# olga24912/lodestar

Hardware: AMD Instinct MI355X
Metric: verified signature sets/sec (node) (higher is better)
Workload: dtype u32/u64 (28-bit-limb Montgomery integer arithmetic); 1 GPU; C2 gossip attestation flood: 16384 single-pubkey sets per GPU, 1 set per batchable job; pk_mode=device table, sig_encoding=compressed 96 B, distinct_messages=16384, group_sets=1024, group_policy=0, inflight=32, slots=3, hw_queues=4, merge_sets=131072, pipeline_depth=3, parallelism=shard-by-job x1 (in-process devices), no collective

## Files before the change

lodestar_amd/build.py:

```python
import hashlib
import os
import subprocess
import sys
import time

PKG = os.path.dirname(os.path.abspath(__file__))
ROOT = os.path.dirname(PKG)
CSRC = os.path.join(PKG, "csrc")
LIB = os.environ.get("BLSGPU_LIB") or os.path.join(PKG, "libblsgpu.so")
ARCH = os.environ.get("BLSGPU_ARCH", "gfx950")
HIPCC = os.environ.get("HIPCC", "/opt/rocm/bin/hipcc")
SOURCES = ["k_sig.hip", "k_msm.hip", "k_hash.hip", "k_hmap.hip", "k_pk.hip", "k_sigagg.hip", "k_awr.hip", "k_same.hip", "k_aggverify.hip", "k_miller.hip", "k_group.hip", "k_inv.hip", "k_ssz.hip", "k_debug.hip", "k_tower_debug.hip",
           "runtime.cpp", "pipeline.cpp", "helpers.cpp"]


OBJ_DIR = os.path.join(PKG, "build")


TU_DEFINES = {"k_sig.hip": ["BLS_INLINE_BIG=1"]}


def tu_defines():
    env = os.environ.get("BLSGPU_TU_DEFINES")
    if env is None:
        return TU_DEFINES
    out = {}
    for part in filter(None, env.split(";")):
        tu, _, defs = part.partition("=")
        out[tu] = [d for d in defs.split("+") if d]
    return out


_ILP = ["-mllvm", "-amdgpu-sched-strategy=max-ilp"]
_MINREG = ["-mllvm", "-amdgpu-sched-strategy=iterative-minreg"]
TU_CFLAGS = {"k_hash.hip": _MINREG, "k_pk.hip": _ILP}


def tu_cflags():
    env = os.environ.get("BLSGPU_TU_CFLAGS")
    if env is None:
        return TU_CFLAGS
    out = {}
# ... 103 lines not shown
```

lodestar_amd/csrc/hash_to_curve.hpp:

```cpp
#pragma once
#include "curve.hpp"

BLS_CONST uint32_t SHA256_K[64] = {
    0x428a2f98, 0x71374491, 0xb5c0fbcf, 0xe9b5dba5, 0x3956c25b, 0x59f111f1, 0x923f82a4, 0xab1c5ed5,
    0xd807aa98, 0x12835b01, 0x243185be, 0x550c7dc3, 0x72be5d74, 0x80deb1fe, 0x9bdc06a7, 0xc19bf174,
    0xe49b69c1, 0xefbe4786, 0x0fc19dc6, 0x240ca1cc, 0x2de92c6f, 0x4a7484aa, 0x5cb0a9dc, 0x76f988da,
    0x983e5152, 0xa831c66d, 0xb00327c8, 0xbf597fc7, 0xc6e00bf3, 0xd5a79147, 0x06ca6351, 0x14292967,
    0x27b70a85, 0x2e1b2138, 0x4d2c6dfc, 0x53380d13, 0x650a7354, 0x766a0abb, 0x81c2c92e, 0x92722c85,
    0xa2bfe8a1, 0xa81a664b, 0xc24b8b70, 0xc76c51a3, 0xd192e819, 0xd6990624, 0xf40e3585, 0x106aa070,
    0x19a4c116, 0x1e376c08, 0x2748774c, 0x34b0bcb5, 0x391c0cb3, 0x4ed8aa4a, 0x5b9cca4f, 0x682e6ff3,
    0x748f82ee, 0x78a5636f, 0x84c87814, 0x8cc70208, 0x90befffa, 0xa4506ceb, 0xbef9a3f7, 0xc67178f2};
BLS_CONST uint32_t SHA256_IV[8] = {0x6a09e667, 0xbb67ae85, 0x3c6ef372, 0xa54ff53a,
                                   0x510e527f, 0x9b05688c, 0x1f83d9ab, 0x5be0cd19};

BLS_HD uint32_t rotr32(uint32_t x, int n) { return (x >> n) | (x << (32 - n)); }

struct sha_st {
  uint32_t h[8];
};
struct sha_blk {
  uint32_t w[16];
};
BLS_HDNI sha_st sha256_block(sha_st st, sha_blk blk) {
  uint32_t a = st.h[0], b = st.h[1], c = st.h[2], d = st.h[3], e = st.h[4], f = st.h[5], g = st.h[6], h = st.h[7];
// ... 106 lines not shown
    int bit = 32 * k;
    int li = bit / BLS_LB, off = bit % BLS_LB;
    lim[li] |= (v << off) & BLS_MASK;
    if (li + 1 < 19) lim[li + 1] |= (off == 0) ? (v >> BLS_LB) : ((v >> (BLS_LB - off)) & BLS_MASK);
    if (off > 0 && li + 2 < 19 && (32 - (BLS_LB - off)) > BLS_LB) lim[li + 2] |= v >> (2 * BLS_LB - off);
  }
  fp lo, hi;
#pragma unroll
  for (int i = 0; i < BLS_NL; i++) lo.l[i] = lim[i];
#pragma unroll
  for (int i = 0; i < BLS_NL; i++) hi.l[i] = (i < 5) ? lim[BLS_NL + i] : 0;
  return fp_add(fp_mul(lo, FP_R2), fp_mul(hi, FP_R3));
}

BLS_INL void hash_to_field_fp2x2(const uint8_t msg[32], fp2& u0, fp2& u1) {
  uint32_t ub[64];
  expand_message_xmd_32(msg, ub);
  u0.c0 = fp_from_be64_words(ub + 0);
  u0.c1 = fp_from_be64_words(ub + 16);
  u1.c0 = fp_from_be64_words(ub + 32);
  u1.c1 = fp_from_be64_words(ub + 48);
}

BLS_INL fp2 fp2_sqrt_with_normroot(const fp2& a, const fp& s) {
  fp t = fp_half(fp_add(a.c0, s));
  fp t_alt = fp_half(fp_sub(a.c0, s));
  t = fp_select(fp_is_zero(t), t_alt, t);
  fp y = fp_pow_p34(t);
  fp x0 = fp_mul(t, y);
  fp a1y2 = fp_half(fp_mul(a.c1, y));
  bool res_case = fp_eq(fp_sqr(x0), t);
  fp2 r;
  r.c0 = fp_select(res_case, x0, a1y2);
  r.c1 = fp_select(res_case, a1y2, fp_neg(x0));
  return r;
}

BLS_HD fp2 fp2_plain(const fp2& a) { return fp2_make(fp_from_mont(a.c0), fp_from_mont(a.c1)); }

BLS_INL g2a sswu_map(const fp2& u, const fp2& Zu2, const fp2& tv, const fp2& tv_inv) {
  fp2 x1 = fp2_mul(SSWU_MINUS_B_OVER_A, fp2_add(fp2_one(), tv_inv));
  x1 = fp2_select(fp2_is_zero(tv), SSWU_B_OVER_ZA, x1);
  fp2 gx1 = fp2_add(fp2_mul(fp2_add(fp2_sqr(x1), SSWU_A), x1), SSWU_B);
  fp2 x2 = fp2_mul(Zu2, x1);
  fp2 gx2 = fp2_add(fp2_mul(fp2_add(fp2_sqr(x2), SSWU_A), x2), SSWU_B);
  fp n1 = fp2_norm(gx1);
  fp s1 = fp_mul(n1, fp_pow_p34(n1));
  bool sq1 = fp_eq(fp_sqr(s1), n1);
  fp nu = fp2_norm(u);
  fp s2 = fp_mul(fp_mul(SSWU_C125, s1), fp_mul(fp_sqr(nu), nu));
  fp2 g = fp2_select(sq1, gx1, gx2);
  fp2 x = fp2_select(sq1, x1, x2);
  fp s = fp_select(sq1, s1, s2);
  fp2 y = fp2_sqrt_with_normroot(g, s);
  fp2 up = fp2_plain(u);
  fp2 yp = fp2_plain(y);
  uint32_t su = fp2_sgn0_plain(up.c0, up.c1);
  uint32_t sy = fp2_sgn0_plain(yp.c0, yp.c1);
  y = fp2_select(su != sy, fp2_neg(y), y);
  g2a r;
  r.x = x;
  r.y = y;
  return r;
}

BLS_INL g2j iso3_map_jac(const g2a& p) {
  const fp2& x = p.x;
  fp2 x2 = fp2_sqr(x);
  fp2 x3 = fp2_mul(x2, x);
  fp2 Nx = fp2_add(fp2_add(fp2_mul(ISO_XNUM_3, x3), fp2_mul(ISO_XNUM_2, x2)), fp2_add(fp2_mul(ISO_XNUM_1, x), ISO_XNUM_0));
  fp2 Dx = fp2_add(fp2_add(x2, fp2_mul(ISO_XDEN_1, x)), ISO_XDEN_0);
  fp2 Ny = fp2_add(fp2_add(fp2_mul(ISO_YNUM_3, x3), fp2_mul(ISO_YNUM_2, x2)), fp2_add(fp2_mul(ISO_YNUM_1, x), ISO_YNUM_0));
  fp2 Dy = fp2_add(fp2_add(x3, fp2_mul(ISO_YDEN_2, x2)), fp2_add(fp2_mul(ISO_YDEN_1, x), ISO_YDEN_0));
  g2j r;
  fp2 DxDy = fp2_mul(Dx, Dy);
  r.z = DxDy;
  r.x = fp2_mul(fp2_mul(Nx, Dy), DxDy);
  fp2 Dx2 = fp2_sqr(Dx);
  r.y = fp2_mul(fp2_mul(fp2_mul(p.y, Ny), fp2_mul(Dx2, Dx)), fp2_sqr(Dy));
  if (fp2_is_zero(DxDy)) r = jac_infinity<fp2>();
  return r;
}

BLS_HDNI g2j clear_cofactor_g2(const g2j& P) {
  g2j t1 = jac_neg(jac_mul_zabs(P));
  g2j t2 = g2_psi(P);
// ... 16 lines not shown
    st(2, jac_add(jac_add(g2_psi2(jac_dbl(P)), jac_neg(psiP)), jac_add(A, jac_neg(P))));
  }
  const jac<F> D = jac_mul_zabs_ld<F>([&] { return ld(1); });
  return jac_add(D, ld(2));
}
template <class Ld, class St>
BLS_INL g2j clear_cofactor_g2_slots(Ld ld, St st) {
  return clear_cofactor_slots<fp2>(ld, st);
}

struct h2c_prep {
  fp2 u0, u1, Zu2_0, Zu2_1, tv0, tv1, d;
};
BLS_INL void hash_to_g2_prep(const uint8_t msg[32], h2c_prep& h) {
  hash_to_field_fp2x2(msg, h.u0, h.u1);
  h.Zu2_0 = fp2_mul(SSWU_Z, fp2_sqr(h.u0));
  h.Zu2_1 = fp2_mul(SSWU_Z, fp2_sqr(h.u1));
  h.tv0 = fp2_add(fp2_sqr(h.Zu2_0), h.Zu2_0);
  h.tv1 = fp2_add(fp2_sqr(h.Zu2_1), h.Zu2_1);
  const fp2 a0 = fp2_select(fp2_is_zero(h.tv0), fp2_one(), h.tv0);
  const fp2 a1 = fp2_select(fp2_is_zero(h.tv1), fp2_one(), h.tv1);
  h.d = fp2_mul(a0, a1);
}
BLS_INL g2j hash_to_g2_map_j(const h2c_prep& h, const fp2& dinv, int j) {
  const bool z0 = fp2_is_zero(h.tv0), z1 = fp2_is_zero(h.tv1);
  const fp2 a_other = j == 0 ? fp2_select(z1, fp2_one(), h.tv1) : fp2_select(z0, fp2_one(), h.tv0);
  const bool zj = j == 0 ? z0 : z1;
  const fp2 inv = fp2_select(zj, fp2_zero(), fp2_mul(dinv, a_other));
  const bool j0 = j == 0;
  const g2a q = sswu_map(fp2_select(j0, h.u0, h.u1), fp2_select(j0, h.Zu2_0, h.Zu2_1), fp2_select(j0, h.tv0, h.tv1), inv);
  return iso3_map_jac(q);
}

BLS_HDNI g2j hash_to_g2_finish(const h2c_prep& h, const fp2& dinv) {
  const bool z0 = fp2_is_zero(h.tv0), z1 = fp2_is_zero(h.tv1);
  const fp2 a0 = fp2_select(z0, fp2_one(), h.tv0);
  const fp2 a1 = fp2_select(z1, fp2_one(), h.tv1);
  const fp2 inv0 = fp2_select(z0, fp2_zero(), fp2_mul(dinv, a1));
  const fp2 inv1 = fp2_select(z1, fp2_zero(), fp2_mul(dinv, a0));
  g2a q0 = sswu_map(h.u0, h.Zu2_0, h.tv0, inv0);
  g2a q1 = sswu_map(h.u1, h.Zu2_1, h.tv1, inv1);
  g2j Q = jac_add(iso3_map_jac(q0), iso3_map_jac(q1));
  return clear_cofactor_g2(Q);
}

BLS_HDNI g2j hash_to_g2_jac(const uint8_t msg[32]) {
  h2c_prep h;
  hash_to_g2_prep(msg, h);
  return hash_to_g2_finish(h, fp2_inv(h.d));
}
```

lodestar_amd/csrc/helpers.cpp:

```cpp
#include "aggverify_plan.hpp"
#include "helper_layout.hpp"
#include "runtime_internal.hpp"

using namespace blsgpu_rt;
namespace hl = helper_layout;
namespace avp = aggverify_plan;

static_assert(hl::kFp == W_FP && hl::kG1A == W_G1A && hl::kG1J == W_G1J && hl::kG2A == W_G2A && hl::kG2J == W_G2J &&
                  hl::kFp12 == W_FP12 && hl::kAwrTabWords == AWR_TAB_WORDS && hl::kMillerLineWords == kMillerLineWords,
              "helper_layout.hpp restates the element widths of kernels.h");

namespace {

template <class Body>
int helper_call(blsgpu_ctx* ctx, bool reads_table, Body body) {
  if (!enter(ctx)) return BLSGPU_ERR_CLOSED;
  struct Leave {
    blsgpu_ctx* ctx;
    ~Leave() { leave(ctx); }
  } leave_on_exit{ctx};
  Device& d = *ctx->devs[0];
  try {
    std::lock_guard<std::mutex> helper(d.helper_mu);
    std::shared_lock<std::shared_mutex> tl(d.table_mu, std::defer_lock);
// ... 803 lines not shown
    HIPCHK(hipGetLastError());
    HIPCHK(hipMemcpyAsync(out32, din + l.out, 32 * (size_t)n, hipMemcpyDeviceToHost, s));
    HIPCHK(hipStreamSynchronize(s));
    return BLSGPU_OK;
  });
}

int blsgpu_debug_op(blsgpu_ctx* ctx, int op, uint32_t n, const uint8_t* in, uint32_t in_stride, uint8_t* out,
                    uint32_t out_stride, int32_t* status) {
  if (!ctx || ctx->devs.empty() || !in || !out || !status) return BLSGPU_ERR_ARGS;
  struct OpSize {
    int op;
    uint32_t in, out;
  };
  static const OpSize kOpSizes[] = {{0, 96, 48},    {1, 194, 192},  {2, 32, 192},   {3, 288, 576},  {4, 576, 576},
                                    {5, 104, 96},   {6, 200, 192},  {7, 64, 96},    {8, 32, 96},    {9, 200, 2880},
                                    {10, 104, 1440}, {11, 840, 56}, {16, 576, 576}, {17, 288, 576}, {18, 384, 192},
      {32, 112, 56}, {33, 56, 56}, {34, 224, 112}, {35, 112, 112}, {36, 168, 112}, {37, 112, 56},
      {38, 112, 56}, {39, 56, 56}, {40, 56, 56}, {41, 56, 56}, {42, 56, 56}, {43, 56, 56},
      {44, 56, 56}, {45, 56, 56}, {46, 112, 56}, {47, 112, 112}, {48, 56, 0}, {49, 112, 0},
      {50, 672, 0}, {51, 56, 56}, {52, 56, 56}, {53, 112, 112}, {54, 336, 336}, {55, 672, 672},
      {56, 112, 112}, {57, 672, 336}, {58, 560, 336}, {59, 560, 336}, {60, 1344, 672}, {61, 672, 672},
      {62, 1008, 672}, {63, 1344, 672}, {64, 672, 672}, {65, 672, 672}, {66, 672, 672}, {67, 672, 672},
      {68, 672, 672}};
  const OpSize* sz = nullptr;
  for (const OpSize& o : kOpSizes)
    if (o.op == op) sz = &o;
  if (!sz || in_stride < sz->in || out_stride < sz->out) return BLSGPU_ERR_ARGS;
  const bool tower = op >= 32;
  if (tower && (in_stride % 4 || out_stride % 4 || out_stride == 0)) return BLSGPU_ERR_ARGS;
  if (n == 0) return BLSGPU_OK;
  return helper_call(ctx, false, [&](Device& d, Slot& sl, hipStream_t s) -> int {
    struct Temp {
      void* p = nullptr;
      ~Temp() {
        if (p) (void)hipFree(p);
      }
    } din, dout, dst;
    HIPCHK(hipMalloc(&din.p, (size_t)n * in_stride));
    HIPCHK(hipMalloc(&dout.p, (size_t)n * out_stride));
    HIPCHK(hipMalloc(&dst.p, (size_t)n * 4));
    HIPCHK(hipMemcpyAsync(din.p, in, (size_t)n * in_stride, hipMemcpyHostToDevice, s));
    HIPCHK(hipMemsetAsync(dout.p, 0, (size_t)n * out_stride, s));
    if (tower)
      launch_debug_tower(op, n, (uint8_t*)din.p, in_stride, (uint8_t*)dout.p, out_stride, (int32_t*)dst.p, s);
    else
      launch_debug_op(op, n, (uint8_t*)din.p, in_stride, (uint8_t*)dout.p, out_stride, (int32_t*)dst.p, s);
    HIPCHK(hipGetLastError());
    HIPCHK(hipMemcpyAsync(out, dout.p, (size_t)n * out_stride, hipMemcpyDeviceToHost, s));
    HIPCHK(hipMemcpyAsync(status, dst.p, (size_t)n * 4, hipMemcpyDeviceToHost, s));
    HIPCHK(hipStreamSynchronize(s));
    return BLSGPU_OK;
  });
}

}
```

lodestar_amd/csrc/k_hmap.hip:

```cpp
#include "k_common.hpp"

#define W_HPREP (7 * 2 * W_FP)

__device__ __forceinline__ void st_prep(uint32_t* p, uint32_t n, uint32_t u, const h2c_prep& h) {
  st_fp2(p, n, u, 0 * W_FP, h.u0);
  st_fp2(p, n, u, 2 * W_FP, h.u1);
  st_fp2(p, n, u, 4 * W_FP, h.Zu2_0);
  st_fp2(p, n, u, 6 * W_FP, h.Zu2_1);
  st_fp2(p, n, u, 8 * W_FP, h.tv0);
  st_fp2(p, n, u, 10 * W_FP, h.tv1);
  st_fp2(p, n, u, 12 * W_FP, h.d);
}
STAGE_KERNEL_W(BLSGPU_WPE_HPREP) void k_hash_prep(PipelineBuffers b) {
  uint32_t u = blockIdx.x * WAVE + threadIdx.x;
  if (u >= b.n_umsg) return;
  uint8_t msg[32];
  const uint4* src = reinterpret_cast<const uint4*>(b.umsgs + (size_t)u * 32);
  uint4 m0 = src[0], m1 = src[1];
  uint32_t w[8] = {m0.x, m0.y, m0.z, m0.w, m1.x, m1.y, m1.z, m1.w};
#pragma unroll
  for (int k = 0; k < 32; k++) msg[k] = (uint8_t)(w[k >> 2] >> (8 * (k & 3)));
  h2c_prep h;
  hash_to_g2_prep(msg, h);
  st_prep(b.h_prep, b.nm, u, h);
// ... 2 lines not shown

__device__ __forceinline__ h2c_prep ld_prep(const uint32_t* p, uint32_t n, uint32_t u) {
  h2c_prep h;
  h.u0 = ld_fp2(p, n, u, 0 * W_FP);
  h.u1 = ld_fp2(p, n, u, 2 * W_FP);
  h.Zu2_0 = ld_fp2(p, n, u, 4 * W_FP);
  h.Zu2_1 = ld_fp2(p, n, u, 6 * W_FP);
  h.tv0 = ld_fp2(p, n, u, 8 * W_FP);
  h.tv1 = ld_fp2(p, n, u, 10 * W_FP);
  h.d = ld_fp2(p, n, u, 12 * W_FP);
  return h;
}

STAGE_KERNEL_W(BLSGPU_WPE_HMAP) void k_hash_map(PipelineBuffers b, const uint32_t* inv) {
  const uint32_t q = blockIdx.x * WAVE + threadIdx.x;
  if (q >= 2 * b.n_umsg) return;
  const uint32_t u = q >> 1, j = q & 1;
  const h2c_prep h = ld_prep(b.h_prep, b.nm, u);
  const fp ni = ld_fp(inv, b.n_umsg, u, 0);
  const fp2 dinv = fp2_make(fp_mul(h.d.c0, ni), fp_neg(fp_mul(h.d.c1, ni)));
  st_g2j(b.h_q, 2 * b.nm, q, hash_to_g2_map_j(h, dinv, (int)j));
}

void launch_hash_prep(const PipelineBuffers& b, hipStream_t s) {
  if (b.n_umsg) hipLaunchKernelGGL(k_hash_prep, dim3((b.n_umsg + WAVE - 1) / WAVE), dim3(WAVE), 0, s, b);
}
void launch_hash_map(const PipelineBuffers& b, const uint32_t* inv, hipStream_t s) {
  if (b.n_umsg) hipLaunchKernelGGL(k_hash_map, dim3((2 * b.n_umsg + WAVE - 1) / WAVE), dim3(WAVE), 0, s, b, inv);
}
```

lodestar_amd/csrc/k_sig.hip:

```cpp
#include "k_common.hpp"
#include "g2_coop.hpp"

#ifndef BLSGPU_SIG_PAIRS
#define BLSGPU_SIG_PAIRS 1
#endif
#ifndef BLSGPU_WPE_DEC0
#define BLSGPU_WPE_DEC0 2
#endif
#ifndef BLSGPU_WPE_SUB2
#define BLSGPU_WPE_SUB2 2
#endif
template <bool CHECK, int WPE>
__global__ __launch_bounds__(WAVE) __attribute__((amdgpu_waves_per_eu(WPE, WPE))) void k_sig_decode(
    PipelineBuffers b, uint32_t n_sets) {
  const bool check_group = CHECK;
  uint32_t i = blockIdx.x * WAVE + threadIdx.x;
  if (i >= n_sets) return;
  uint8_t raw[192];
  uint32_t len = b.sig_len[i];
  const uint8_t* src = b.sigs + (size_t)i * b.sig_stride;
  uint32_t cl = len == 96 || len == 192 ? len : 0;
  for (uint32_t k = 0; k < cl; k++) raw[k] = src[k];
  g2a p;
  bool inf = false;
  int st = sig_decode_point(raw, len, p, inf);
  if (st != BLS_OK || inf) {
    p.x = fp2_zero();
    p.y = fp2_zero();
  }
  st_g2a(b.sig_aff, b.n, i, p);
  if (check_group && st == BLS_OK && !inf &&
      !g2_in_subgroup_ld([&] { return ld_g2a(b.sig_aff, b.n, opaque_u32(i)); })) {
    st = BLS_POINT_NOT_IN_GROUP;
    p.x = fp2_zero();
    p.y = fp2_zero();
    st_g2a(b.sig_aff, b.n, i, p);
  }
  b.flags[i] = inf ? SF_SIG_INF : 0;
  b.status[i] = (int8_t)st;
}

STAGE_KERNEL_W(BLSGPU_WPE_SUB2) void k_sig_subgroup2(PipelineBuffers b, uint32_t n_sets) {
  const uint32_t q = blockIdx.x * WAVE + threadIdx.x, i = q >> 1, k = q & 1;
  if (i >= n_sets || b.status[i] != BLS_OK || (b.flags[i] & SF_SIG_INF)) return;
  auto ldP = [&] {
    const uint32_t ii = opaque_u32(i);
    aff<fp2x> a;
    a.x.v = ld_fp(b.sig_aff, b.n, ii, (int)(k * W_FP));
    a.y.v = ld_fp(b.sig_aff, b.n, ii, (int)((2 + k) * W_FP));
    return a;
  };
  const g2jx zP = jac_neg(jac_mul_zabs_lda<fp2x>(ldP));
  if (!jac_eq(g2_psi(jac_from_aff(ldP())), zP)) {
    st_fp(b.sig_aff, b.n, i, (int)(k * W_FP), fp_zero());
    st_fp(b.sig_aff, b.n, i, (int)((2 + k) * W_FP), fp_zero());
    if (k == 0) b.status[i] = (int8_t)BLS_POINT_NOT_IN_GROUP;
  }
}

STAGE_KERNEL void k_sig_scale(PipelineBuffers b, uint32_t n_sets, const uint32_t* list) {
  const uint32_t q = blockIdx.x * WAVE + threadIdx.x;
  if (q >= n_sets) return;
// ... 20 lines not shown
  if (tg == 0 && on) {
    const g2j zP = jac_neg(g2c_ld_point(g));
    if (!jac_eq(g2_psi(jac_from_aff(ld_g2a(b.sig_aff, b.n, i))), zP)) {
      g2a z;
      z.x = fp2_zero();
      z.y = fp2_zero();
      st_g2a(b.sig_aff, b.n, i, z);
      b.status[i] = (int8_t)BLS_POINT_NOT_IN_GROUP;
    }
  }
}

__global__ __launch_bounds__(WAVE) void k_spec_mask(PipelineBuffers b, uint32_t n_sets, uint8_t* spec) {
  const uint32_t i = blockIdx.x * WAVE + threadIdx.x;
  if (i < n_sets) spec[i] = b.status[i] == BLS_OK ? 1 : 0;
}

static inline dim3 grid_for(uint32_t n) { return dim3((n + WAVE - 1) / WAVE); }

void launch_spec_mask(const PipelineBuffers& b, uint32_t n, uint8_t* spec, hipStream_t s) {
  if (n) hipLaunchKernelGGL(k_spec_mask, grid_for(n), dim3(WAVE), 0, s, b, n, spec);
}

void launch_sig_decode(const PipelineBuffers& b, uint32_t n, hipStream_t s, bool coop, hipEvent_t decoded,
                       bool exclusive, bool subgroup) {
  if (!n) return;
  if (!subgroup) {
    hipLaunchKernelGGL((k_sig_decode<false, BLSGPU_WPE_DEC0>), grid_for(n), dim3(WAVE), 0, s, b, n);
    if (decoded) (void)hipEventRecord(decoded, s);
    return;
  }
  if (coop || BLSGPU_SIG_PAIRS)
    hipLaunchKernelGGL((k_sig_decode<false, BLSGPU_WPE_DEC0>), grid_for(n), dim3(WAVE), 0, s, b, n);
  else
    hipLaunchKernelGGL((k_sig_decode<true, BLSGPU_WPE_DEC>), grid_for(n), dim3(WAVE), 0, s, b, n);
  if (decoded) (void)hipEventRecord(decoded, s);
  if (!coop) {
    if (BLSGPU_SIG_PAIRS) hipLaunchKernelGGL(k_sig_subgroup2, grid_for(2 * n), dim3(WAVE), 0, s, b, n);
  } else
    hipLaunchKernelGGL(k_sig_subgroup_coop, dim3((n + SG_GROUPS - 1) / SG_GROUPS), dim3(WAVE),
                       BLSGPU_EXCLUSIVE_SMALL && exclusive ? exclusive_cu_lds<k_sig_subgroup_coop>() : 0, s, b, n);
}
void launch_sig_scale(const PipelineBuffers& b, uint32_t n, hipStream_t s, const uint32_t* list) {
  if (n) hipLaunchKernelGGL(k_sig_scale, grid_for(n), dim3(WAVE), 0, s, b, n, list);
}
```

lodestar_amd/csrc/kernels.h:

```cpp
#pragma once
#include <hip/hip_runtime.h>
#include <stdint.h>
#include <vector>

#define W_FP 14
#define W_G1A (2 * W_FP)
#define W_G1J (3 * W_FP)
#define W_G2A (4 * W_FP)
#define W_G2J (6 * W_FP)
#define W_FP12 (12 * W_FP)
#define W_PKTAB 32
#define MILLER_STEPS 68
#define W_LINE (3 * 2 * W_FP)

#define SF_SIG_INF 1u
#define MF_H_INF 1u

struct PipelineBuffers {
  uint32_t n;
  const uint8_t* sigs;
  const uint32_t* sig_len;
  uint32_t sig_stride;
  const uint8_t* pk_bytes;
  const uint32_t* set_pk_first;
// ... 25 lines not shown
  uint32_t* inv_buf_pk;
  uint32_t* pk_jac;
  uint32_t* pk_aff;
  uint32_t* rsig;
  uint32_t* unit_p;
  uint32_t n_chunks;
  const uint32_t* chunk_first;
  const uint32_t* chunk_items;
  uint32_t* f_chunk;
  uint32_t* lines;
  uint8_t* flags;
  uint8_t* mflags;
  uint8_t* unit_ok;
  int8_t* status;
  int8_t* job_err;
  uint8_t* include;
};

void launch_sig_decode(const PipelineBuffers& b, uint32_t n_sets, hipStream_t s, bool coop = false,
                       hipEvent_t decoded = nullptr, bool exclusive = true, bool subgroup = true);
void launch_spec_mask(const PipelineBuffers& b, uint32_t n_sets, uint8_t* spec, hipStream_t s);
void launch_hash_prep(const PipelineBuffers& b, hipStream_t s);
void launch_hash_map(const PipelineBuffers& b, const uint32_t* inv, hipStream_t s);
void launch_hash_to_g2(const PipelineBuffers& b, hipStream_t s, bool coop = false,
                       bool exclusive = true);
void launch_pk_aggregate(const PipelineBuffers& b, uint32_t n_sets, hipStream_t s);
void launch_pk_finish(const PipelineBuffers& b, uint32_t n_sets, hipStream_t s);
void launch_batch_inv(const uint32_t* src, uint32_t src_stride, int w0, uint32_t* dst, uint32_t n, hipStream_t s);
void launch_pk_affine(const PipelineBuffers& b, uint32_t n_sets, hipStream_t s);
void launch_h_affine(const PipelineBuffers& b, hipStream_t s);
void launch_sig_scale(const PipelineBuffers& b, uint32_t n_sets, hipStream_t s, const uint32_t* list = nullptr);
#ifndef MSM_SLICE
#define MSM_SLICE 256
#endif
#define MSM_BUCKET_WORDS (128 * W_G2J)
#define MSM_WINDOW_WORDS (16 * W_G2J)
void launch_sig_msm(const PipelineBuffers& b, const uint32_t* slices, uint32_t n_slices, const uint32_t* range_slices,
                    uint32_t n_ranges, uint32_t* B, uint32_t* W, uint32_t* S, hipStream_t s, bool lane_tail = false,
                    uint32_t tree_slices = 0);
void launch_job_mask(const PipelineBuffers& b, hipStream_t s);
void launch_unit_aggregate(const PipelineBuffers& b, hipStream_t s);
void launch_miller_lines(const PipelineBuffers& b, hipStream_t s);
void launch_miller_lines2(const PipelineBuffers& b, hipStream_t s);
void launch_miller_accx(const PipelineBuffers& b, bool units, hipStream_t s);
#define MILLER_MAX_SEGS 8
struct MillerSegs {
// ... 153 lines not shown
```

lodestar_amd/csrc/ops.hpp:

```cpp
#pragma once
#include "hash_to_curve.hpp"
#include "pairing.hpp"

enum {
  BLS_OK = 0,
  BLS_BAD_ENCODING = 1,
  BLS_POINT_NOT_ON_CURVE = 2,
  BLS_POINT_NOT_IN_GROUP = 3,
  BLS_AGGR_TYPE_MISMATCH = 4,
  BLS_VERIFY_FAIL = 5,
  BLS_PK_IS_INFINITY = 6,
  BLS_BAD_SCALAR = 7,
  BLS_INVALID_SIZE = 8,
  BLS_EMPTY_AGGREGATE = 9,
  BLS_EMPTY_SET = 10,
  BLS_DEVICE_ERROR = 11,
};

BLS_HD bool bytes_all_zero(const uint8_t* b, int n) {
  uint32_t o = 0;
  for (int i = 0; i < n; i++) o |= b[i];
  return o == 0;
}

BLS_HDNI int sig_decode_point(const uint8_t* b, uint32_t len, g2a& out, bool& inf) {
  inf = false;
  if (len != 96 && len != 192) return BLS_INVALID_SIZE;
  const uint8_t b0 = b[0];
  const bool compressed = (b0 & 0x80) != 0;
  if (compressed != (len == 96)) return BLS_BAD_ENCODING;
  if (b0 & 0x40) {
    if ((b0 & 0x3f) == 0 && bytes_all_zero(b + 1, (int)len - 1)) {
      inf = true;
      return BLS_OK;
    }
    return BLS_BAD_ENCODING;
  }
  fp x1, x0;
  bool ok1 = fp_from_be48_plain(b, x1, 0x1f);
  bool ok0 = fp_from_be48_plain(b + 48, x0, 0xff);
  if (compressed) {
    if (!ok1 || !ok0) return BLS_BAD_ENCODING;
    g2a p;
    p.x = fp2_make(fp_to_mont(x0), fp_to_mont(x1));
    fp2 rhs = fp2_add(fp2_mul(fp2_sqr(p.x), p.x), FP2_B2);
    fp2 y;
    if (!fp2_sqrt(rhs, y)) return BLS_POINT_NOT_ON_CURVE;
    fp2 yp = fp2_plain(y);
    bool c1z = fp_is_zero(yp.c1);
    bool largest = c1z ? fp_plain_gt_half(yp.c0) : fp_plain_gt_half(yp.c1);
    bool want = (b0 & 0x20) != 0;
    p.y = fp2_select(largest != want, fp2_neg(y), y);
    out = p;
  } else {
    if (b0 & 0x20) return BLS_BAD_ENCODING;
    fp y1, y0;
    bool ok3 = fp_from_be48_plain(b + 96, y1, 0xff);
    bool ok2 = fp_from_be48_plain(b + 144, y0, 0xff);
    if (!ok1 || !ok0 || !ok2 || !ok3) return BLS_BAD_ENCODING;
    g2a p;
    p.x = fp2_make(fp_to_mont(x0), fp_to_mont(x1));
    p.y = fp2_make(fp_to_mont(y0), fp_to_mont(y1));
    if (!g2_on_curve(p)) return BLS_POINT_NOT_ON_CURVE;
    out = p;
  }
  return BLS_OK;
}
BLS_HDNI int sig_decode(const uint8_t* b, uint32_t len, g2a& out, bool& inf) {
  const int st = sig_decode_point(b, len, out, inf);
  if (st != BLS_OK || inf) return st;
  return g2_in_subgroup(out) ? BLS_OK : BLS_POINT_NOT_IN_GROUP;
}

BLS_HDNI int pk_decode96(const uint8_t* b, g1a& out, bool& inf) {
  inf = false;
  const uint8_t b0 = b[0];
  if (b0 & 0x80) return BLS_BAD_ENCODING;
  if (b0 & 0x40) {
    if ((b0 & 0x3f) == 0 && bytes_all_zero(b + 1, 95)) {
      inf = true;
      return BLS_OK;
    }
    return BLS_BAD_ENCODING;
  }
  if (b0 & 0x20) return BLS_BAD_ENCODING;
  fp x, y;
  bool okx = fp_from_be48_plain(b, x, 0xff);
  bool oky = fp_from_be48_plain(b + 48, y, 0xff);
// ... 80 lines not shown
```

lodestar_amd/csrc/runtime.cpp:

```cpp
#include <pthread.h>
#include <stdio.h>
#include <sys/random.h>

#include <system_error>

#include "call_plan.hpp"
#include "runtime_internal.hpp"

using namespace blsgpu_rt;

namespace {

thread_local bool tl_dispatcher = false;

}

namespace blsgpu_rt __attribute__((visibility("hidden"))) {

struct Owned {
  std::vector<uint32_t> jfs, siglen, pkfirst, pkidx;
  std::vector<uint8_t> jflags, pkb, msgs, sigs;
};

struct Call {
// ... 572 lines not shown
extern "C" {

int blsgpu_init(const int* devices, int n_devices, blsgpu_ctx** out) {
  if (!out) return BLSGPU_ERR_ARGS;
  *out = nullptr;
  int count = 0;
  if (hipGetDeviceCount(&count) != hipSuccess || count <= 0) return BLSGPU_ERR_NO_DEVICE;
  std::vector<int> ids;
  if (devices && n_devices > 0) {
    for (int i = 0; i < n_devices; i++) {
      if (devices[i] < 0 || devices[i] >= count) return BLSGPU_ERR_ARGS;
      ids.push_back(devices[i]);
    }
  } else {
    for (int i = 0; i < count; i++) ids.push_back(i);
  }
  blsgpu_ctx* ctx = new blsgpu_ctx();
  ctx->hw_queues = hw_queues_of_process();
  ctx->slots_per_device = default_slots(ctx->hw_queues);
  if (const char* v = getenv("BLSGPU_MILLER_SEGMENTS")) {
    const long j = strtol(v, nullptr, 10);
    if (j >= 1 && j <= MILLER_MAX_SEGS) ctx->opt.miller_segments = j;
  }
  try {
    for (int id : ids) {
      Device* d = new Device();
      d->id = id;
      ctx->devs.push_back(d);
      HIPCHK(hipSetDevice(id));
      HIPCHK(hipStreamCreateWithFlags(&d->table_stream, hipStreamNonBlocking));
    }
  } catch (HipError&) {
    blsgpu_destroy(ctx);
    return BLSGPU_ERR_NO_DEVICE;
  }
  *out = ctx;
  return BLSGPU_OK;
}

void blsgpu_destroy(blsgpu_ctx* ctx) {
  if (!ctx) return;
  {
    std::unique_lock<std::mutex> lk(ctx->active_mu);
    ctx->closed = true;
    ctx->active_cv.wait(lk, [&] { return ctx->active == 0; });
  }
// ... 396 lines not shown
```

lodestar_amd/csrc/tower.hpp:

```cpp
#pragma once
#include "fp.hpp"

struct fp6 {
  fp2 c0, c1, c2;
};
struct fp12 {
  fp6 c0, c1;
};

BLS_HD fp2 fp2_make(const fp& a, const fp& b) {
  fp2 r;
  r.c0 = a;
  r.c1 = b;
  return r;
}
BLS_HD fp2 fp2_zero() { return fp2_make(fp_zero(), fp_zero()); }
BLS_HD fp2 fp2_one() { return fp2_make(FP_ONE, fp_zero()); }
BLS_FN fp2 fp2_add(const fp2& a, const fp2& b) { return fp2_make(fp_add(a.c0, b.c0), fp_add(a.c1, b.c1)); }
BLS_FN fp2 fp2_sub(const fp2& a, const fp2& b) { return fp2_make(fp_sub(a.c0, b.c0), fp_sub(a.c1, b.c1)); }
BLS_HD fp2 fp2_neg(const fp2& a) { return fp2_make(fp_neg(a.c0), fp_neg(a.c1)); }
BLS_HD fp2 fp2_dbl(const fp2& a) { return fp2_make(fp_dbl(a.c0), fp_dbl(a.c1)); }
BLS_HD fp2 fp2_half(const fp2& a) { return fp2_make(fp_half(a.c0), fp_half(a.c1)); }
BLS_HD fp2 fp2_conj(const fp2& a) { return fp2_make(a.c0, fp_neg(a.c1)); }
BLS_HD fp2 fp2_add_nr(const fp2& a, const fp2& b) { return fp2_make(fp_add_nr(a.c0, b.c0), fp_add_nr(a.c1, b.c1)); }
// ... 211 lines not shown
  BLS_COUNT(bls_count_mul);
  return fp2_sqr_body(a);
}
#endif


BLS_FN fp2 fp2_mul_xi(const fp2& a) { return fp2_make(fp_sub(a.c0, a.c1), fp_add(a.c0, a.c1)); }

BLS_FN fp2 fp2_mul3(const fp2& a) { return fp2_make(fp_mul3(a.c0), fp_mul3(a.c1)); }

BLS_FN bool fp2_is_zero(const fp2& a) { return fp_is_zero(a.c0) && fp_is_zero(a.c1); }
BLS_FN bool fp2_eq(const fp2& a, const fp2& b) { return fp_eq(a.c0, b.c0) && fp_eq(a.c1, b.c1); }
BLS_HD fp2 fp2_select(bool c, const fp2& a, const fp2& b) {
  return fp2_make(fp_select(c, a.c0, b.c0), fp_select(c, a.c1, b.c1));
}
BLS_FN fp fp2_norm(const fp2& a) {
  return fp_add(fp_sqr(a.c0), fp_sqr(a.c1));
}
BLS_FN fp2 fp2_inv(const fp2& a) {
  fp ni = fp_inv(fp2_norm(a));
  return fp2_make(fp_mul(a.c0, ni), fp_neg(fp_mul(a.c1, ni)));
}

BLS_HDNI bool fp2_sqrt(const fp2& a, fp2& out) {
  fp n = fp2_norm(a);
  fp e1 = fp_pow_p34(n);
  fp s = fp_mul(n, e1);
  bool ok = fp_eq(fp_sqr(s), n);
  fp t = fp_half(fp_add(a.c0, s));
  fp t_alt = fp_half(fp_sub(a.c0, s));
  t = fp_select(fp_is_zero(t), t_alt, t);
  fp y = fp_pow_p34(t);
  fp x0 = fp_mul(t, y);
  fp a1y2 = fp_half(fp_mul(a.c1, y));
  bool res_case = fp_eq(fp_sqr(x0), t);
  fp2 r;
  r.c0 = fp_select(res_case, x0, a1y2);
  r.c1 = fp_select(res_case, a1y2, fp_neg(x0));
  out = r;
  bool check = fp2_eq(fp2_sqr(r), a);
  return ok && check;
}

BLS_HD uint32_t fp2_sgn0_plain(const fp& c0, const fp& c1) {
  uint32_t s0 = c0.l[0] & 1u;
  uint32_t z0 = 1;
  for (int i = 0; i < BLS_NL; i++) z0 &= (c0.l[i] == 0);
  uint32_t s1 = c1.l[0] & 1u;
  return s0 | (z0 & s1);
}

BLS_HD fp6 fp6_make(const fp2& a, const fp2& b, const fp2& c) {
  fp6 r;
  r.c0 = a;
  r.c1 = b;
  r.c2 = c;
  return r;
}
BLS_HD fp6 fp6_zero() { return fp6_make(fp2_zero(), fp2_zero(), fp2_zero()); }
BLS_HD fp6 fp6_one() { return fp6_make(fp2_one(), fp2_zero(), fp2_zero()); }
BLS_FN fp6 fp6_add(const fp6& a, const fp6& b) { return fp6_make(fp2_add(a.c0, b.c0), fp2_add(a.c1, b.c1), fp2_add(a.c2, b.c2)); }
// ... 351 lines not shown
```

Before: 4.294 million sets/s.

## Split Fp2 square-root exponentiations into standalone pow kernels for large batches

Breaks the hash-to-curve SSWU map and compressed-signature decompression into three-stage kernel chains. The two p-3/4 exponentiations of each Fp2 sqrt now run in a dedicated lean k_pow_p34 kernel, with intermediate state spilled to the existing h_q and sig_aff buffers. The aim is to keep the heavy exponentiation out of register-hungry fused kernels so it runs at higher occupancy. In exchange it adds extra launches and global-memory round trips. The split only applies when the lane count reaches a threshold (default 65536, overridable by environment variable); below that the original fused kernels run.

```diff
diff --git a/lodestar_amd/build.py b/lodestar_amd/build.py
--- a/lodestar_amd/build.py
+++ b/lodestar_amd/build.py
@@ -10,14 +10,14 @@
 LIB = os.environ.get("BLSGPU_LIB") or os.path.join(PKG, "libblsgpu.so")
 ARCH = os.environ.get("BLSGPU_ARCH", "gfx950")
 HIPCC = os.environ.get("HIPCC", "/opt/rocm/bin/hipcc")
-SOURCES = ["k_sig.hip", "k_msm.hip", "k_hash.hip", "k_hmap.hip", "k_pk.hip", "k_sigagg.hip", "k_awr.hip", "k_same.hip", "k_aggverify.hip", "k_miller.hip", "k_group.hip", "k_inv.hip", "k_ssz.hip", "k_debug.hip", "k_tower_debug.hip",
+SOURCES = ["k_sig.hip", "k_msm.hip", "k_hash.hip", "k_hmap.hip", "k_pow.hip", "k_pk.hip", "k_sigagg.hip", "k_awr.hip", "k_same.hip", "k_aggverify.hip", "k_miller.hip", "k_group.hip", "k_inv.hip", "k_ssz.hip", "k_debug.hip", "k_tower_debug.hip",
            "runtime.cpp", "pipeline.cpp", "helpers.cpp"]
 
 
 OBJ_DIR = os.path.join(PKG, "build")
 
 
-TU_DEFINES = {"k_sig.hip": ["BLS_INLINE_BIG=1"]}
+TU_DEFINES = {"k_sig.hip": ["BLS_INLINE_BIG=1"], "k_pow.hip": ["BLS_INLINE_BIG=1"]}
 
 
 def tu_defines():
diff --git a/lodestar_amd/csrc/hash_to_curve.hpp b/lodestar_amd/csrc/hash_to_curve.hpp
--- a/lodestar_amd/csrc/hash_to_curve.hpp
+++ b/lodestar_amd/csrc/hash_to_curve.hpp
@@ -152,37 +152,32 @@
   u1.c1 = fp_from_be64_words(ub + 48);
 }
 
-BLS_INL fp2 fp2_sqrt_with_normroot(const fp2& a, const fp& s) {
-  fp t = fp_half(fp_add(a.c0, s));
-  fp t_alt = fp_half(fp_sub(a.c0, s));
-  t = fp_select(fp_is_zero(t), t_alt, t);
-  fp y = fp_pow_p34(t);
-  fp x0 = fp_mul(t, y);
-  fp a1y2 = fp_half(fp_mul(a.c1, y));
-  bool res_case = fp_eq(fp_sqr(x0), t);
-  fp2 r;
-  r.c0 = fp_select(res_case, x0, a1y2);
-  r.c1 = fp_select(res_case, a1y2, fp_neg(x0));
-  return r;
-}
-
 BLS_HD fp2 fp2_plain(const fp2& a) { return fp2_make(fp_from_mont(a.c0), fp_from_mont(a.c1)); }
 
-BLS_INL g2a sswu_map(const fp2& u, const fp2& Zu2, const fp2& tv, const fp2& tv_inv) {
+BLS_INL fp2 sswu_g(const fp2& x) { return fp2_add(fp2_mul(fp2_add(fp2_sqr(x), SSWU_A), x), SSWU_B); }
+BLS_INL fp2 sswu_x1(const fp2& tv, const fp2& tv_inv) {
   fp2 x1 = fp2_mul(SSWU_MINUS_B_OVER_A, fp2_add(fp2_one(), tv_inv));
-  x1 = fp2_select(fp2_is_zero(tv), SSWU_B_OVER_ZA, x1);
-  fp2 gx1 = fp2_add(fp2_mul(fp2_add(fp2_sqr(x1), SSWU_A), x1), SSWU_B);
+  return fp2_select(fp2_is_zero(tv), SSWU_B_OVER_ZA, x1);
+}
+struct sswu_mid {
+  fp2 x, g;
+  fp t;
+};
+BLS_INL sswu_mid sswu_map_mid(const fp2& u, const fp2& Zu2, const fp2& x1, const fp2& gx1, const fp& n1, const fp& e1) {
   fp2 x2 = fp2_mul(Zu2, x1);
-  fp2 gx2 = fp2_add(fp2_mul(fp2_add(fp2_sqr(x2), SSWU_A), x2), SSWU_B);
-  fp n1 = fp2_norm(gx1);
-  fp s1 = fp_mul(n1, fp_pow_p34(n1));
-  bool sq1 = fp_eq(fp_sqr(s1), n1);
+  fp2 gx2 = sswu_g(x2);
+  bool sq1;
+  fp s1 = fp2_sqrt_norm_root(n1, e1, sq1);
   fp nu = fp2_norm(u);
   fp s2 = fp_mul(fp_mul(SSWU_C125, s1), fp_mul(fp_sqr(nu), nu));
-  fp2 g = fp2_select(sq1, gx1, gx2);
-  fp2 x = fp2_select(sq1, x1, x2);
-  fp s = fp_select(sq1, s1, s2);
-  fp2 y = fp2_sqrt_with_normroot(g, s);
+  sswu_mid m;
+  m.g = fp2_select(sq1, gx1, gx2);
+  m.x = fp2_select(sq1, x1, x2);
+  m.t = fp2_sqrt_t(m.g, fp_select(sq1, s1, s2));
+  return m;
+}
+BLS_INL g2a sswu_map_end(const fp2& u, const fp2& x, const fp2& g, const fp& t, const fp& yt) {
+  fp2 y = fp2_sqrt_root(g, t, yt);
   fp2 up = fp2_plain(u);
   fp2 yp = fp2_plain(y);
   uint32_t su = fp2_sgn0_plain(up.c0, up.c1);
@@ -192,6 +187,13 @@
   r.x = x;
   r.y = y;
   return r;
+}
+BLS_INL g2a sswu_map(const fp2& u, const fp2& Zu2, const fp2& tv, const fp2& tv_inv) {
+  const fp2 x1 = sswu_x1(tv, tv_inv);
+  const fp2 gx1 = sswu_g(x1);
+  const fp n1 = fp2_norm(gx1);
+  const sswu_mid m = sswu_map_mid(u, Zu2, x1, gx1, n1, fp_pow_p34(n1));
+  return sswu_map_end(u, m.x, m.g, m.t, fp_pow_p34(m.t));
 }
 
 BLS_INL g2j iso3_map_jac(const g2a& p) {
@@ -254,13 +256,15 @@
   const fp2 a1 = fp2_select(fp2_is_zero(h.tv1), fp2_one(), h.tv1);
   h.d = fp2_mul(a0, a1);
 }
+BLS_INL fp2 h2c_map_inv(const fp2& tv_j, const fp2& tv_other, const fp2& dinv) {
+  const fp2 a_other = fp2_select(fp2_is_zero(tv_other), fp2_one(), tv_other);
+  return fp2_select(fp2_is_zero(tv_j), fp2_zero(), fp2_mul(dinv, a_other));
+}
 BLS_INL g2j hash_to_g2_map_j(const h2c_prep& h, const fp2& dinv, int j) {
-  const bool z0 = fp2_is_zero(h.tv0), z1 = fp2_is_zero(h.tv1);
-  const fp2 a_other = j == 0 ? fp2_select(z1, fp2_one(), h.tv1) : fp2_select(z0, fp2_one(), h.tv0);
-  const bool zj = j == 0 ? z0 : z1;
-  const fp2 inv = fp2_select(zj, fp2_zero(), fp2_mul(dinv, a_other));
   const bool j0 = j == 0;
-  const g2a q = sswu_map(fp2_select(j0, h.u0, h.u1), fp2_select(j0, h.Zu2_0, h.Zu2_1), fp2_select(j0, h.tv0, h.tv1), inv);
+  const fp2 tv_j = fp2_select(j0, h.tv0, h.tv1);
+  const fp2 inv = h2c_map_inv(tv_j, fp2_select(j0, h.tv1, h.tv0), dinv);
+  const g2a q = sswu_map(fp2_select(j0, h.u0, h.u1), fp2_select(j0, h.Zu2_0, h.Zu2_1), tv_j, inv);
   return iso3_map_jac(q);
 }
 
diff --git a/lodestar_amd/csrc/helpers.cpp b/lodestar_amd/csrc/helpers.cpp
--- a/lodestar_amd/csrc/helpers.cpp
+++ b/lodestar_amd/csrc/helpers.cpp
@@ -849,11 +849,13 @@
       {50, 672, 0}, {51, 56, 56}, {52, 56, 56}, {53, 112, 112}, {54, 336, 336}, {55, 672, 672},
       {56, 112, 112}, {57, 672, 336}, {58, 560, 336}, {59, 560, 336}, {60, 1344, 672}, {61, 672, 672},
       {62, 1008, 672}, {63, 1344, 672}, {64, 672, 672}, {65, 672, 672}, {66, 672, 672}, {67, 672, 672},
-      {68, 672, 672}};
+      {68, 672, 672},
+      {19, 56, 56}};
   const OpSize* sz = nullptr;
   for (const OpSize& o : kOpSizes)
     if (o.op == op) sz = &o;
   if (!sz || in_stride < sz->in || out_stride < sz->out) return BLSGPU_ERR_ARGS;
+  if (op == 19 && (in_stride != 56 || out_stride != 56)) return BLSGPU_ERR_ARGS;
   const bool tower = op >= 32;
   if (tower && (in_stride % 4 || out_stride % 4 || out_stride == 0)) return BLSGPU_ERR_ARGS;
   if (n == 0) return BLSGPU_OK;
@@ -869,7 +871,10 @@
     HIPCHK(hipMalloc(&dst.p, (size_t)n * 4));
     HIPCHK(hipMemcpyAsync(din.p, in, (size_t)n * in_stride, hipMemcpyHostToDevice, s));
     HIPCHK(hipMemsetAsync(dout.p, 0, (size_t)n * out_stride, s));
-    if (tower)
+    if (op == 19) {
+      HIPCHK(hipMemsetAsync(dst.p, 0, (size_t)n * 4, s));
+      launch_pow_p34((const uint32_t*)din.p, 0, (uint32_t*)dout.p, 0, n, n, s);
+    } else if (tower)
       launch_debug_tower(op, n, (uint8_t*)din.p, in_stride, (uint8_t*)dout.p, out_stride, (int32_t*)dst.p, s);
     else
       launch_debug_op(op, n, (uint8_t*)din.p, in_stride, (uint8_t*)dout.p, out_stride, (int32_t*)dst.p, s);
diff --git a/lodestar_amd/csrc/k_hmap.hip b/lodestar_amd/csrc/k_hmap.hip
--- a/lodestar_amd/csrc/k_hmap.hip
+++ b/lodestar_amd/csrc/k_hmap.hip
@@ -48,9 +48,62 @@
   st_g2j(b.h_q, 2 * b.nm, q, hash_to_g2_map_j(h, dinv, (int)j));
 }
 
+#define HQ_POW_IN 0
+#define HQ_POW_OUT W_FP
+#define HQ_X (2 * W_FP)
+#define HQ_G (4 * W_FP)
+static_assert(HQ_G + 2 * W_FP <= W_G2J, "the split maps' state fits the lane's h_q entry");
+__device__ __forceinline__ fp2 ld_prep_j(const PipelineBuffers& b, uint32_t u, uint32_t k, uint32_t j) {
+  return ld_fp2(b.h_prep, b.nm, u, (int)((2 * k + j) * 2 * W_FP));
+}
+STAGE_KERNEL_W(BLSGPU_WPE_HMAP) void k_hash_map_a(PipelineBuffers b, const uint32_t* inv) {
+  const uint32_t q = blockIdx.x * WAVE + threadIdx.x;
+  if (q >= 2 * b.n_umsg) return;
+  const uint32_t u = q >> 1, j = q & 1, qs = 2 * b.nm;
+  const fp2 d = ld_fp2(b.h_prep, b.nm, u, 12 * W_FP);
+  const fp ni = ld_fp(inv, b.n_umsg, u, 0);
+  const fp2 dinv = fp2_make(fp_mul(d.c0, ni), fp_neg(fp_mul(d.c1, ni)));
+  const fp2 tv_j = ld_prep_j(b, u, 2, j);
+  const fp2 x1 = sswu_x1(tv_j, h2c_map_inv(tv_j, ld_prep_j(b, u, 2, j ^ 1), dinv));
+  const fp2 gx1 = sswu_g(x1);
+  st_fp(b.h_q, qs, q, HQ_POW_IN, fp2_norm(gx1));
+  st_fp2(b.h_q, qs, q, HQ_X, x1);
+  st_fp2(b.h_q, qs, q, HQ_G, gx1);
+}
+STAGE_KERNEL_W(BLSGPU_WPE_HMAP) void k_hash_map_b(PipelineBuffers b) {
+  const uint32_t q = blockIdx.x * WAVE + threadIdx.x;
+  if (q >= 2 * b.n_umsg) return;
+  const uint32_t u = q >> 1, j = q & 1, qs = 2 * b.nm;
+  const sswu_mid m = sswu_map_mid(ld_prep_j(b, u, 0, j), ld_prep_j(b, u, 1, j), ld_fp2(b.h_q, qs, q, HQ_X),
+                                  ld_fp2(b.h_q, qs, q, HQ_G), ld_fp(b.h_q, qs, q, HQ_POW_IN),
+                                  ld_fp(b.h_q, qs, q, HQ_POW_OUT));
+  st_fp(b.h_q, qs, q, HQ_POW_IN, m.t);
+  st_fp2(b.h_q, qs, q, HQ_X, m.x);
+  st_fp2(b.h_q, qs, q, HQ_G, m.g);
+}
+STAGE_KERNEL_W(BLSGPU_WPE_HMAP) void k_hash_map_c(PipelineBuffers b) {
+  const uint32_t q = blockIdx.x * WAVE + threadIdx.x;
+  if (q >= 2 * b.n_umsg) return;
+  const uint32_t u = q >> 1, j = q & 1, qs = 2 * b.nm;
+  const g2a p = sswu_map_end(ld_prep_j(b, u, 0, j), ld_fp2(b.h_q, qs, q, HQ_X), ld_fp2(b.h_q, qs, q, HQ_G),
+                             ld_fp(b.h_q, qs, q, HQ_POW_IN), ld_fp(b.h_q, qs, q, HQ_POW_OUT));
+  st_g2j(b.h_q, qs, q, iso3_map_jac(p));
+}
+
 void launch_hash_prep(const PipelineBuffers& b, hipStream_t s) {
   if (b.n_umsg) hipLaunchKernelGGL(k_hash_prep, dim3((b.n_umsg + WAVE - 1) / WAVE), dim3(WAVE), 0, s, b);
 }
 void launch_hash_map(const PipelineBuffers& b, const uint32_t* inv, hipStream_t s) {
-  if (b.n_umsg) hipLaunchKernelGGL(k_hash_map, dim3((2 * b.n_umsg + WAVE - 1) / WAVE), dim3(WAVE), 0, s, b, inv);
+  if (!b.n_umsg) return;
+  const uint32_t lanes = 2 * b.n_umsg;
+  const dim3 grid((lanes + WAVE - 1) / WAVE);
+  if (!pow_split(lanes)) {
+    hipLaunchKernelGGL(k_hash_map, grid, dim3(WAVE), 0, s, b, inv);
+    return;
+  }
+  hipLaunchKernelGGL(k_hash_map_a, grid, dim3(WAVE), 0, s, b, inv);
+  launch_pow_p34(b.h_q, HQ_POW_IN, b.h_q, HQ_POW_OUT, 2 * b.nm, lanes, s);
+  hipLaunchKernelGGL(k_hash_map_b, grid, dim3(WAVE), 0, s, b);
+  launch_pow_p34(b.h_q, HQ_POW_IN, b.h_q, HQ_POW_OUT, 2 * b.nm, lanes, s);
+  hipLaunchKernelGGL(k_hash_map_c, grid, dim3(WAVE), 0, s, b);
 }
diff --git a/lodestar_amd/csrc/k_pow.hip b/lodestar_amd/csrc/k_pow.hip
--- /dev/null
+++ b/lodestar_amd/csrc/k_pow.hip
@@ -0,0 +1,18 @@
+#include <atomic>
+
+#include "k_common.hpp"
+
+STAGE_KERNEL_W(4) void k_pow_p34(const uint32_t* in, int w_in, uint32_t* out, int w_out, uint32_t stride, uint32_t n) {
+  const uint32_t i = blockIdx.x * WAVE + threadIdx.x;
+  if (i >= n) return;
+  st_fp(out, stride, i, w_out, fp_pow_p34(ld_fp(in, stride, i, w_in)));
+}
+
+void launch_pow_p34(const uint32_t* in, int w_in, uint32_t* out, int w_out, uint32_t stride, uint32_t n,
+                    hipStream_t s) {
+  if (n) hipLaunchKernelGGL(k_pow_p34, dim3((n + WAVE - 1) / WAVE), dim3(WAVE), 0, s, in, w_in, out, w_out, stride, n);
+}
+
+static std::atomic<uint32_t> g_pow_split_lanes{POW_SPLIT_LANES};
+void set_pow_split_lanes(uint32_t lanes) { g_pow_split_lanes.store(lanes ? lanes : POW_SPLIT_LANES); }
+bool pow_split(uint64_t lanes) { return lanes >= g_pow_split_lanes.load(std::memory_order_relaxed); }
diff --git a/lodestar_amd/csrc/k_sig.hip b/lodestar_amd/csrc/k_sig.hip
--- a/lodestar_amd/csrc/k_sig.hip
+++ b/lodestar_amd/csrc/k_sig.hip
@@ -38,6 +38,70 @@
   }
   b.flags[i] = inf ? SF_SIG_INF : 0;
   b.status[i] = (int8_t)st;
+}
+
+#define SA_POW_IN (2 * W_FP)
+#define SA_POW_OUT (3 * W_FP)
+__device__ __forceinline__ bool sig_open(const PipelineBuffers& b, uint32_t i) {
+  return b.status[i] == BLS_OK && b.sig_len[i] == 96 && !(b.flags[i] & SF_SIG_INF);
+}
+__device__ __forceinline__ void sig_reject(const PipelineBuffers& b, uint32_t i, int st) {
+  g2a z;
+  z.x = fp2_zero();
+  z.y = fp2_zero();
+  st_g2a(b.sig_aff, b.n, i, z);
+  b.status[i] = (int8_t)st;
+}
+STAGE_KERNEL_W(BLSGPU_WPE_DEC0) void k_sig_decode_a(PipelineBuffers b, uint32_t n_sets) {
+  uint32_t i = blockIdx.x * WAVE + threadIdx.x;
+  if (i >= n_sets) return;
+  uint8_t raw[192];
+  uint32_t len = b.sig_len[i];
+  const uint8_t* src = b.sigs + (size_t)i * b.sig_stride;
+  uint32_t cl = len == 96 || len == 192 ? len : 0;
+  for (uint32_t k = 0; k < cl; k++) raw[k] = src[k];
+  g2a p;
+  bool inf = false, need_y = false;
+  int st = sig_decode_head(raw, len, p, inf, need_y);
+  if (st != BLS_OK || inf) p.x = fp2_zero();
+  p.y = fp2_zero();
+  if (need_y) p.y.c0 = fp2_norm(sig_curve_rhs(p.x));
+  st_g2a(b.sig_aff, b.n, i, p);
+  b.flags[i] = inf ? SF_SIG_INF : 0;
+  b.status[i] = (int8_t)st;
+}
+STAGE_KERNEL_W(BLSGPU_WPE_DEC0) void k_sig_decode_b(PipelineBuffers b, uint32_t n_sets) {
+  uint32_t i = blockIdx.x * WAVE + threadIdx.x;
+  if (i >= n_sets || !sig_open(b, i)) return;
+  const fp2 rhs = sig_curve_rhs(ld_fp2(b.sig_aff, b.n, i, 0));
+  bool ok;
+  const fp s = fp2_sqrt_norm_root(ld_fp(b.sig_aff, b.n, i, SA_POW_IN), ld_fp(b.sig_aff, b.n, i, SA_POW_OUT), ok);
+  if (!ok) {
+    sig_reject(b, i, BLS_POINT_NOT_ON_CURVE);
+    return;
+  }
+  st_fp(b.sig_aff, b.n, i, SA_POW_IN, fp2_sqrt_t(rhs, s));
+}
+STAGE_KERNEL_W(BLSGPU_WPE_DEC0) void k_sig_decode_c(PipelineBuffers b, uint32_t n_sets) {
+  uint32_t i = blockIdx.x * WAVE + threadIdx.x;
+  if (i >= n_sets) return;
+  const uint8_t* src = b.sigs + (size_t)i * b.sig_stride;
+  fp2 y = fp2_zero();
+  if (sig_open(b, i)) {
+    const fp2 rhs = sig_curve_rhs(ld_fp2(b.sig_aff, b.n, i, 0));
+    const fp2 r = fp2_sqrt_root(rhs, ld_fp(b.sig_aff, b.n, i, SA_POW_IN), ld_fp(b.sig_aff, b.n, i, SA_POW_OUT));
+    if (!fp2_eq(fp2_sqr(r), rhs)) {
+      sig_reject(b, i, BLS_POINT_NOT_ON_CURVE);
+      return;
+    }
+    y = sig_decode_pick_y(r, src[0]);
+  } else if (b.status[i] == BLS_OK && b.sig_len[i] == 192 && !(b.flags[i] & SF_SIG_INF)) {
+    fp y1, y0;
+    (void)fp_from_be48_plain(src + 96, y1, 0xff);
+    (void)fp_from_be48_plain(src + 144, y0, 0xff);
+    y = fp2_make(fp_to_mont(y0), fp_to_mont(y1));
+  }
+  st_fp2(b.sig_aff, b.n, i, 2 * W_FP, y);
 }
 
 STAGE_KERNEL_W(BLSGPU_WPE_SUB2) void k_sig_subgroup2(PipelineBuffers b, uint32_t n_sets) {
@@ -104,16 +168,28 @@
   if (n) hipLaunchKernelGGL(k_spec_mask, grid_for(n), dim3(WAVE), 0, s, b, n, spec);
 }
 
+static void launch_point_decode(const PipelineBuffers& b, uint32_t n, hipStream_t s) {
+  if (!pow_split(n)) {
+    hipLaunchKernelGGL((k_sig_decode<false, BLSGPU_WPE_DEC0>), grid_for(n), dim3(WAVE), 0, s, b, n);
+    return;
+  }
+  hipLaunchKernelGGL(k_sig_decode_a, grid_for(n), dim3(WAVE), 0, s, b, n);
+  launch_pow_p34(b.sig_aff, SA_POW_IN, b.sig_aff, SA_POW_OUT, b.n, n, s);
+  hipLaunchKernelGGL(k_sig_decode_b, grid_for(n), dim3(WAVE), 0, s, b, n);
+  launch_pow_p34(b.sig_aff, SA_POW_IN, b.sig_aff, SA_POW_OUT, b.n, n, s);
+  hipLaunchKernelGGL(k_sig_decode_c, grid_for(n), dim3(WAVE), 0, s, b, n);
+}
+
 void launch_sig_decode(const PipelineBuffers& b, uint32_t n, hipStream_t s, bool coop, hipEvent_t decoded,
                        bool exclusive, bool subgroup) {
   if (!n) return;
   if (!subgroup) {
-    hipLaunchKernelGGL((k_sig_decode<false, BLSGPU_WPE_DEC0>), grid_for(n), dim3(WAVE), 0, s, b, n);
+    launch_point_decode(b, n, s);
     if (decoded) (void)hipEventRecord(decoded, s);
     return;
   }
   if (coop || BLSGPU_SIG_PAIRS)
-    hipLaunchKernelGGL((k_sig_decode<false, BLSGPU_WPE_DEC0>), grid_for(n), dim3(WAVE), 0, s, b, n);
+    launch_point_decode(b, n, s);
   else
     hipLaunchKernelGGL((k_sig_decode<true, BLSGPU_WPE_DEC>), grid_for(n), dim3(WAVE), 0, s, b, n);
   if (decoded) (void)hipEventRecord(decoded, s);
diff --git a/lodestar_amd/csrc/kernels.h b/lodestar_amd/csrc/kernels.h
--- a/lodestar_amd/csrc/kernels.h
+++ b/lodestar_amd/csrc/kernels.h
@@ -71,6 +71,11 @@
 void launch_spec_mask(const PipelineBuffers& b, uint32_t n_sets, uint8_t* spec, hipStream_t s);
 void launch_hash_prep(const PipelineBuffers& b, hipStream_t s);
 void launch_hash_map(const PipelineBuffers& b, const uint32_t* inv, hipStream_t s);
+void launch_pow_p34(const uint32_t* in, int w_in, uint32_t* out, int w_out, uint32_t stride, uint32_t n,
+                    hipStream_t s);
+#define POW_SPLIT_LANES 65536u
+void set_pow_split_lanes(uint32_t lanes);
+bool pow_split(uint64_t lanes);
 void launch_hash_to_g2(const PipelineBuffers& b, hipStream_t s, bool coop = false,
                        bool exclusive = true);
 void launch_pk_aggregate(const PipelineBuffers& b, uint32_t n_sets, hipStream_t s);
diff --git a/lodestar_amd/csrc/ops.hpp b/lodestar_amd/csrc/ops.hpp
--- a/lodestar_amd/csrc/ops.hpp
+++ b/lodestar_amd/csrc/ops.hpp
@@ -23,8 +23,17 @@
   return o == 0;
 }
 
-BLS_HDNI int sig_decode_point(const uint8_t* b, uint32_t len, g2a& out, bool& inf) {
+BLS_INL fp2 sig_curve_rhs(const fp2& x) { return fp2_add(fp2_mul(fp2_sqr(x), x), FP2_B2); }
+BLS_INL fp2 sig_decode_pick_y(const fp2& y, uint8_t b0) {
+  fp2 yp = fp2_plain(y);
+  bool c1z = fp_is_zero(yp.c1);
+  bool largest = c1z ? fp_plain_gt_half(yp.c0) : fp_plain_gt_half(yp.c1);
+  bool want = (b0 & 0x20) != 0;
+  return fp2_select(largest != want, fp2_neg(y), y);
+}
+BLS_INL int sig_decode_head(const uint8_t* b, uint32_t len, g2a& out, bool& inf, bool& need_y) {
   inf = false;
+  need_y = false;
   if (len != 96 && len != 192) return BLS_INVALID_SIZE;
   const uint8_t b0 = b[0];
   const bool compressed = (b0 & 0x80) != 0;
@@ -41,17 +50,8 @@
   bool ok0 = fp_from_be48_plain(b + 48, x0, 0xff);
   if (compressed) {
     if (!ok1 || !ok0) return BLS_BAD_ENCODING;
-    g2a p;
-    p.x = fp2_make(fp_to_mont(x0), fp_to_mont(x1));
-    fp2 rhs = fp2_add(fp2_mul(fp2_sqr(p.x), p.x), FP2_B2);
-    fp2 y;
-    if (!fp2_sqrt(rhs, y)) return BLS_POINT_NOT_ON_CURVE;
-    fp2 yp = fp2_plain(y);
-    bool c1z = fp_is_zero(yp.c1);
-    bool largest = c1z ? fp_plain_gt_half(yp.c0) : fp_plain_gt_half(yp.c1);
-    bool want = (b0 & 0x20) != 0;
-    p.y = fp2_select(largest != want, fp2_neg(y), y);
-    out = p;
+    out.x = fp2_make(fp_to_mont(x0), fp_to_mont(x1));
+    need_y = true;
   } else {
     if (b0 & 0x20) return BLS_BAD_ENCODING;
     fp y1, y0;
@@ -64,6 +64,19 @@
     if (!g2_on_curve(p)) return BLS_POINT_NOT_ON_CURVE;
     out = p;
   }
+  return BLS_OK;
+}
+BLS_HDNI int sig_decode_point(const uint8_t* b, uint32_t len, g2a& out, bool& inf) {
+  bool need_y;
+  g2a p;
+  const int st = sig_decode_head(b, len, p, inf, need_y);
+  if (st != BLS_OK || inf) return st;
+  if (need_y) {
+    fp2 y;
+    if (!fp2_sqrt(sig_curve_rhs(p.x), y)) return BLS_POINT_NOT_ON_CURVE;
+    p.y = sig_decode_pick_y(y, b[0]);
+  }
+  out = p;
   return BLS_OK;
 }
 BLS_HDNI int sig_decode(const uint8_t* b, uint32_t len, g2a& out, bool& inf) {
diff --git a/lodestar_amd/csrc/runtime.cpp b/lodestar_amd/csrc/runtime.cpp
--- a/lodestar_amd/csrc/runtime.cpp
+++ b/lodestar_amd/csrc/runtime.cpp
@@ -618,6 +618,11 @@
     const long j = strtol(v, nullptr, 10);
     if (j >= 1 && j <= MILLER_MAX_SEGS) ctx->opt.miller_segments = j;
   }
+  {
+    const char* v = getenv("BLSGPU_POW_SPLIT_LANES");
+    const long l = v ? strtol(v, nullptr, 10) : 0;
+    set_pow_split_lanes(l >= 1 && l <= 0x7fffffffL ? (uint32_t)l : 0);
+  }
   try {
     for (int id : ids) {
       Device* d = new Device();
diff --git a/lodestar_amd/csrc/tower.hpp b/lodestar_amd/csrc/tower.hpp
--- a/lodestar_amd/csrc/tower.hpp
+++ b/lodestar_amd/csrc/tower.hpp
@@ -257,21 +257,31 @@
   return fp2_make(fp_mul(a.c0, ni), fp_neg(fp_mul(a.c1, ni)));
 }
 
-BLS_HDNI bool fp2_sqrt(const fp2& a, fp2& out) {
-  fp n = fp2_norm(a);
-  fp e1 = fp_pow_p34(n);
+BLS_FN fp fp2_sqrt_norm_root(const fp& n, const fp& e1, bool& ok) {
   fp s = fp_mul(n, e1);
-  bool ok = fp_eq(fp_sqr(s), n);
+  ok = fp_eq(fp_sqr(s), n);
+  return s;
+}
+BLS_FN fp fp2_sqrt_t(const fp2& a, const fp& s) {
   fp t = fp_half(fp_add(a.c0, s));
   fp t_alt = fp_half(fp_sub(a.c0, s));
-  t = fp_select(fp_is_zero(t), t_alt, t);
-  fp y = fp_pow_p34(t);
+  return fp_select(fp_is_zero(t), t_alt, t);
+}
+BLS_FN fp2 fp2_sqrt_root(const fp2& a, const fp& t, const fp& y) {
   fp x0 = fp_mul(t, y);
   fp a1y2 = fp_half(fp_mul(a.c1, y));
   bool res_case = fp_eq(fp_sqr(x0), t);
   fp2 r;
   r.c0 = fp_select(res_case, x0, a1y2);
   r.c1 = fp_select(res_case, a1y2, fp_neg(x0));
+  return r;
+}
+BLS_HDNI bool fp2_sqrt(const fp2& a, fp2& out) {
+  fp n = fp2_norm(a);
+  bool ok;
+  fp s = fp2_sqrt_norm_root(n, fp_pow_p34(n), ok);
+  fp t = fp2_sqrt_t(a, s);
+  fp2 r = fp2_sqrt_root(a, t, fp_pow_p34(t));
   out = r;
   bool check = fp2_eq(fp2_sqr(r), a);
   return ok && check;
```

Measured after the change: 4.238 million sets/s. 1.3% lower.
